# kuetuofa/Transformer

Measured on AMD Instinct MI355X. Metric: tokens/sec (whole node), Transformer-base NMT training, higher is better.
Workload: dtype bf16; 1 GPU; model=transformer-base, num_layers=6, d_model=512, num_heads=8, dff=2048, global_batch=64, seq_len=256, vocab=32770, parallelism=dp1

## Files before the change

transformer_amd/ops/csrc/gemm256.hip:

```cpp
#include "common.h"

#include <torch/extension.h>
#include <ATen/hip/HIPContext.h>

typedef __bf16 bf16x8g __attribute__((ext_vector_type(8)));

namespace {

#define G_BM 256
#define G_BK 64
#define G_THREADS 512
#define G_TILE_ELEMS (G_BM * G_BK)

DEV_INLINE int sw256(int off) { return off ^ (((off >> 9) & 1) << 5); }

template <int ROWS = 256>
DEV_INLINE void stage256(const short* __restrict__ g, long ldg, int row0,
                         int maxrow, int h, short* lds) {
  const int wid = threadIdx.x >> 6, lane = threadIdx.x & 63;
#pragma unroll
  for (int p = 0; p < ROWS / 128; ++p) {
    const int chunk = h * (ROWS / 16) + p * 8 + wid;
    const int d = chunk * 1024 + lane * 16;
    const int lg = sw256(d);
    int row = row0 + (lg >> 7);
    if (row > maxrow - 1) row = maxrow - 1;
    const int colb = lg & 127;
    __builtin_amdgcn_global_load_lds(
        (const __attribute__((address_space(1))) void*)(g + (long)row * ldg +
                                                        (colb >> 1)),
        (__attribute__((address_space(3))) void*)((char*)lds + d), 16, 0, 0);
  }
}

DEV_INLINE bf16x8g frag256(const short* lds, int row, int kb ) {
  const int off = sw256(row * 128 + kb);
  return (bf16x8g)*(const s16x8*)((const char*)lds + off);
}

#define G_BARRIER() __builtin_amdgcn_s_barrier()
#define G_WAIT_LGKM0() asm volatile("s_waitcnt lgkmcnt(0)" ::: "memory")
#define G_WAIT_VM0() asm volatile("s_waitcnt vmcnt(0)" ::: "memory")

template <int EPILOGUE, int BM_, int BN_, int ORDER = 0, int XCDMAP = 1>
__global__ __launch_bounds__(G_THREADS, 1)
void gemm256_kernel(const short* __restrict__ A, const short* __restrict__ B,
                    const short* __restrict__ bias, short* __restrict__ C,
                    int M, int N, int K, int lda, int ldb, int has_bias,
                    int nbm, int nbn, const short* __restrict__ aux) {
  constexpr int MF = BM_ / 32;
  constexpr int NF = BN_ / 64;
  constexpr int A_ELEMS = BM_ * G_BK;
  constexpr int B_ELEMS = BN_ * G_BK;
  constexpr int SLOT = A_ELEMS + B_ELEMS;
  extern __shared__ short smem[];
  const int lane = threadIdx.x & 63;

  int nwg = nbm * nbn;
  int wg = blockIdx.x;
  if (XCDMAP) {
    int q = nwg / 8, r = nwg % 8, x = wg % 8, o = wg / 8;
    wg = (x < r ? x * (q + 1) : r * (q + 1) + (x - r) * q) + o;
  }
  const int bm0 = (ORDER ? (wg % nbm) : (wg / nbn)) * BM_;
  const int bn0 = (ORDER ? (wg / nbm) : (wg % nbn)) * BN_;

  const int wid = threadIdx.x >> 6;
  const int wm = (wid >> 2) * (BM_ / 2);
  const int wn = (wid & 3) * (BN_ / 4);
  const int fr = lane & 15;
  const int kg = lane >> 4;

  f32x4 acc[MF][NF];
#pragma unroll
  for (int i = 0; i < MF; ++i)
#pragma unroll
    for (int j = 0; j < NF; ++j) acc[i][j] = {0.f, 0.f, 0.f, 0.f};

  const int ntiles = K / G_BK;

  {
    short* a0 = smem;
    short* b0 = smem + A_ELEMS;
#pragma unroll
    for (int h = 0; h < 2; ++h) {
      stage256<BM_>(A, lda, bm0, M, h, a0);
      stage256<BN_>(B, ldb, bn0, N, h, b0);
    }
  }
  G_WAIT_VM0();
  G_BARRIER();

  bf16x8g afr[MF / 2][2], bfr[NF][2];

  for (int t = 0; t < ntiles; ++t) {
    const short* a_lds = smem + (t & 1) * SLOT;
    const short* b_lds = a_lds + A_ELEMS;
    short* pa_lds = smem + ((t + 1) & 1) * SLOT;
    short* pb_lds = pa_lds + A_ELEMS;
    const long pk0 = (long)(t + 1) * G_BK;
    const bool do_pf = t + 1 < ntiles;

#define G_MFMA_QUAD(RH, CH)                                                \
  _Pragma("unroll") for (int ks = 0; ks < 2; ++ks)                         \
    _Pragma("unroll") for (int i = 0; i < MF / 2; ++i)                     \
      _Pragma("unroll") for (int j = 0; j < NF / 2; ++j)                   \
        acc[(RH) * (MF / 2) + i][(CH) * (NF / 2) + j] =                    \
            __builtin_amdgcn_mfma_f32_16x16x32_bf16(                       \
                afr[i][ks], bfr[(CH) * (NF / 2) + j][ks],                  \
                acc[(RH) * (MF / 2) + i][(CH) * (NF / 2) + j], 0, 0, 0);

#pragma unroll
    for (int i = 0; i < MF / 2; ++i)
#pragma unroll
      for (int ks = 0; ks < 2; ++ks)
        afr[i][ks] = frag256(a_lds, wm + i * 16 + fr, ks * 64 + kg * 16);
#pragma unroll
    for (int j = 0; j < NF / 2; ++j)
#pragma unroll
      for (int ks = 0; ks < 2; ++ks)
        bfr[j][ks] = frag256(b_lds, wn + j * 16 + fr, ks * 64 + kg * 16);
    if (do_pf) {
      stage256<BM_>(A + pk0, lda, bm0, M, 0, pa_lds);
      stage256<BM_>(A + pk0, lda, bm0, M, 1, pa_lds);
    }
    G_WAIT_LGKM0();
    G_MFMA_QUAD(0, 0)

#pragma unroll
    for (int j = NF / 2; j < NF; ++j)
#pragma unroll
      for (int ks = 0; ks < 2; ++ks)
        bfr[j][ks] = frag256(b_lds, wn + j * 16 + fr, ks * 64 + kg * 16);
    if (do_pf) {
      stage256<BN_>(B + pk0, ldb, bn0, N, 0, pb_lds);
      stage256<BN_>(B + pk0, ldb, bn0, N, 1, pb_lds);
    }
    G_WAIT_LGKM0();
    G_MFMA_QUAD(0, 1)

#pragma unroll
    for (int i = 0; i < MF / 2; ++i)
#pragma unroll
      for (int ks = 0; ks < 2; ++ks)
        afr[i][ks] = frag256(a_lds, wm + (BM_ / 4) + i * 16 + fr,
                             ks * 64 + kg * 16);
    G_WAIT_LGKM0();
    G_MFMA_QUAD(1, 0)

    G_MFMA_QUAD(1, 1)
    G_WAIT_VM0();
    G_BARRIER();
#undef G_MFMA_QUAD
  }

#pragma unroll
  for (int i = 0; i < MF; ++i) {
    const int grow_base = bm0 + wm + i * 16 + kg * 4;
#pragma unroll
    for (int j = 0; j < NF; ++j) {
      const int gcol = bn0 + wn + j * 16 + fr;
      if (gcol >= N) continue;
      const float bv = (has_bias && bias) ? bfbits2f(bias[gcol]) : 0.0f;
#pragma unroll
      for (int r = 0; r < 4; ++r) {
        const int grow = grow_base + r;
        if (grow >= M) continue;
        float v = acc[i][j][r] + bv;
        if (EPILOGUE == 1) v = fmaxf(v, 0.0f);
        if (EPILOGUE == 3) v += bfbits2f(aux[(long)grow * N + gcol]);
        short o = f2bfbits(v);
        if (EPILOGUE == 2)
          o = bfbits2f(aux[(long)grow * N + gcol]) > 0.f ? o : (short)0;
        C[(long)grow * N + gcol] = o;
      }
    }
  }
}

}

static void gemm256_tile(int M, int N, int& BM, int& BN) {
  const long g22 = (long)cdiv(M, 256) * cdiv(N, 256);
  const long g21 = (long)cdiv(M, 256) * cdiv(N, 128);
  auto util = [](long nwg) {
    return nwg < 1 ? 0.0 : (double)nwg / ((nwg + 255) / 256 * 256);
  };
  if (g22 >= 224) {
    BM = 256;
    BN = (util(g21) > util(g22) + 0.1) ? 128 : 256;
  }
  else if (g21 >= 224) { BM = 256; BN = 128; }
  else { BM = 128; BN = 128; }
}

bool gemm256_viable(int M, int N, int K, int lda, int ldb) {
  if (K % G_BK != 0 || K < 2 * G_BK) return false;
  if (lda % 8 != 0 || ldb % 8 != 0) return false;
  int BM, BN;
  gemm256_tile(M, N, BM, BN);
  long nwg = (long)cdiv(M, BM) * cdiv(N, BN);
  return nwg >= 224 && (K >= 512 || nwg >= 384);
}

torch::Tensor gemm256_nt(torch::Tensor a, torch::Tensor w, torch::Tensor bias,
                         int64_t epilogue, c10::optional<torch::Tensor> out,
                         c10::optional<torch::Tensor> aux) {
  TORCH_CHECK(a.is_cuda() && a.dtype() == torch::kBFloat16 && a.dim() == 2 &&
              a.is_contiguous(), "gemm256_nt: a must be contiguous bf16 2-D");
  TORCH_CHECK(w.is_cuda() && w.dtype() == torch::kBFloat16 && w.dim() == 2 &&
              w.is_contiguous(), "gemm256_nt: w must be contiguous bf16 2-D");
  const int M = a.size(0), K = a.size(1), N = w.size(0);
  TORCH_CHECK(w.size(1) == K, "gemm256_nt: K mismatch");
  TORCH_CHECK(K % G_BK == 0 && K >= 2 * G_BK,
              "gemm256_nt: K must be a multiple of 64 (>=128)");
  TORCH_CHECK(epilogue >= 0 && epilogue <= 3, "gemm256_nt: bad epilogue");
  const bool has_bias = epilogue < 2 && bias.defined() && bias.numel() > 0;
  const short* auxp = nullptr;
  if (epilogue >= 2) {
    TORCH_CHECK(aux.has_value() && aux->is_cuda() &&
                aux->dtype() == torch::kBFloat16 && aux->dim() == 2 &&
                aux->is_contiguous() && aux->size(0) == M &&
                aux->size(1) == N,
                "gemm256_nt: epilogue 2/3 needs a contiguous bf16 (M, N) aux");
    TORCH_CHECK(!(bias.defined() && bias.numel() > 0),
                "gemm256_nt: epilogue 2/3 takes no bias");
    auxp = (const short*)aux->data_ptr();
  }
  torch::Tensor c;
  if (out.has_value()) {
    c = *out;
    TORCH_CHECK(c.is_cuda() && c.dtype() == torch::kBFloat16 &&
                c.is_contiguous() && c.numel() == (long)M * N,
                "out must be contiguous bf16 with M*N elements");
    TORCH_CHECK(!auxp || c.data_ptr() != (void*)auxp,
                "gemm256_nt: out must not alias aux");
  } else {
    c = torch::empty({M, N}, a.options());
  }
  int BMv, BNv;
  gemm256_tile(M, N, BMv, BNv);
  const int nbm = cdiv(M, BMv), nbn = cdiv(N, BNv);
  const size_t smem = 2 * ((size_t)BMv + BNv) * G_BK * sizeof(short);
  auto stream = at::hip::getCurrentHIPStream();
  static bool attr_set[4][3] = {};
  static const int env_order = [] {
    const char* e = getenv("TFMX_G256_ORDER");
    return e ? (e[0] == 'n' ? 1 : 0) : -1;
  }();
  static const int env_xcd = [] {
    const char* e = getenv("TFMX_G256_XCD");
    return e ? atoi(e) : -1;
  }();
  const int order = env_order >= 0 ? env_order : 0;
  const int xcd = env_xcd >= 0 ? env_xcd : 1;
  auto launch = [&](auto epi, auto bmc, auto bnc) {
    constexpr int E = decltype(epi)::value;
    constexpr int BM_ = decltype(bmc)::value;
    constexpr int BN_ = decltype(bnc)::value;
    constexpr int ti = BM_ == 128 ? 2 : (BN_ == 128 ? 1 : 0);
    auto go = [&](auto oc, auto xc) {
      constexpr int OV = decltype(oc)::value;
      constexpr int XV = decltype(xc)::value;
      if (!attr_set[E][ti]) {
        (void)hipFuncSetAttribute(
            (const void*)gemm256_kernel<E, BM_, BN_, OV, XV>,
            hipFuncAttributeMaxDynamicSharedMemorySize, (int)smem);
        attr_set[E][ti] = true;
      }
      gemm256_kernel<E, BM_, BN_, OV, XV>
          <<<nbm * nbn, G_THREADS, smem, stream>>>(
              (const short*)a.data_ptr(), (const short*)w.data_ptr(),
              has_bias ? (const short*)bias.data_ptr() : nullptr,
              (short*)c.data_ptr(), M, N, K, K, K, has_bias, nbm, nbn,
              auxp);
    };
    using I0 = std::integral_constant<int, 0>;
    using I1 = std::integral_constant<int, 1>;
    if (order) { if (xcd) go(I1{}, I1{}); else go(I1{}, I0{}); }
    else       { if (xcd) go(I0{}, I1{}); else go(I0{}, I0{}); }
  };
  using E0 = std::integral_constant<int, 0>;
  using E1 = std::integral_constant<int, 1>;
  using E2 = std::integral_constant<int, 2>;
  using E3 = std::integral_constant<int, 3>;
  using T256 = std::integral_constant<int, 256>;
  using T128 = std::integral_constant<int, 128>;
  auto dis = [&](auto epi) {
    if (BMv == 128) launch(epi, T128{}, T128{});
    else if (BNv == 128) launch(epi, T256{}, T128{});
    else launch(epi, T256{}, T256{});
  };
  if (epilogue == 3) dis(E3{});
  else if (epilogue == 2) dis(E2{});
  else if (epilogue == 1) dis(E1{});
  else dis(E0{});
  return c;
}
```

Baseline: 1.868 million tokens/s.

## Vectorize GEMM epilogue via transposed MFMA and LDS-staged 16-byte stores

Swaps the MFMA operand order so each lane holds four consecutive output columns, then writes the epilogue with packed vector stores. By default (aligned, N%8==0) the fragments are staged through a swizzled per-wave LDS slice and written back as 16-byte row-contiguous stores, with bias and aux loads vectorized too. This targets the scalar 2-byte strided global stores of the old epilogue. The cost is extra LDS traffic, more register pressure and more template instances, with a scalar fallback for unaligned shapes.

```diff
diff --git a/transformer_amd/ops/csrc/gemm256.hip b/transformer_amd/ops/csrc/gemm256.hip
--- a/transformer_amd/ops/csrc/gemm256.hip
+++ b/transformer_amd/ops/csrc/gemm256.hip
@@ -1,4 +1,7 @@
 #include "common.h"
+
+#include <cstdint>
+#include <cstring>
 
 #include <torch/extension.h>
 #include <ATen/hip/HIPContext.h>
@@ -38,16 +41,104 @@
   return (bf16x8g)*(const s16x8*)((const char*)lds + off);
 }
 
+DEV_INLINE unsigned pk_bf16(float lo, float hi) {
+  return (unsigned)(unsigned short)f2bfbits(lo) |
+         ((unsigned)(unsigned short)f2bfbits(hi) << 16);
+}
+
+template <int VEC>
+DEV_INLINE f32x4 epi_bias4(const short* __restrict__ bias, int gcol, int N) {
+  f32x4 bv = {0.f, 0.f, 0.f, 0.f};
+  if (bias && gcol < N) {
+    if (VEC == 8) {
+      const s16x4 b = *(const s16x4*)(bias + gcol);
+#pragma unroll
+      for (int r = 0; r < 4; ++r) bv[r] = bfbits2f(b[r]);
+    } else {
+#pragma unroll
+      for (int r = 0; r < 4; ++r)
+        if (gcol + r < N) bv[r] = bfbits2f(bias[gcol + r]);
+    }
+  }
+  return bv;
+}
+
+template <int EPILOGUE, int VEC>
+DEV_INLINE s16x4 epi_frag_value(f32x4 a, f32x4 bv,
+                                const short* __restrict__ aux, long idx,
+                                int gcol, int N) {
+  s16x4 ax = {0, 0, 0, 0};
+  if (EPILOGUE >= 2) {
+    if (VEC == 8) {
+      ax = *(const s16x4*)(aux + idx);
+    } else if (VEC == 2) {
+      const s16x2 lo = *(const s16x2*)(aux + idx);
+      ax[0] = lo[0]; ax[1] = lo[1];
+      if (gcol + 2 < N) {
+        const s16x2 hi = *(const s16x2*)(aux + idx + 2);
+        ax[2] = hi[0]; ax[3] = hi[1];
+      }
+    } else {
+#pragma unroll
+      for (int r = 0; r < 4; ++r)
+        if (gcol + r < N) ax[r] = aux[idx + r];
+    }
+  }
+  float v[4];
+#pragma unroll
+  for (int r = 0; r < 4; ++r) {
+    v[r] = a[r] + bv[r];
+    if (EPILOGUE == 1) v[r] = fmaxf(v[r], 0.0f);
+    if (EPILOGUE == 3) v[r] += bfbits2f(ax[r]);
+  }
+  union { unsigned u[2]; s16x4 s; } o;
+  o.u[0] = pk_bf16(v[0], v[1]);
+  o.u[1] = pk_bf16(v[2], v[3]);
+  if (EPILOGUE == 2) {
+#pragma unroll
+    for (int r = 0; r < 4; ++r)
+      o.s[r] = bfbits2f(ax[r]) > 0.f ? o.s[r] : (short)0;
+  }
+  return o.s;
+}
+
+template <int VEC>
+DEV_INLINE void epi_frag_store(short* __restrict__ C, long idx, int gcol,
+                               int N, s16x4 o) {
+  if (VEC == 8) {
+    *(s16x4*)(C + idx) = o;
+  } else if (VEC == 2) {
+    *(s16x2*)(C + idx) = s16x2{o[0], o[1]};
+    if (gcol + 2 < N) *(s16x2*)(C + idx + 2) = s16x2{o[2], o[3]};
+  } else {
+#pragma unroll
+    for (int r = 0; r < 4; ++r)
+      if (gcol + r < N) C[idx + r] = o[r];
+  }
+}
+
+template <int CW>
+DEV_INLINE int epi_slot16(int row, int q) {
+  return CW == 64 ? row * 128 + ((q ^ (row & 7)) << 4)
+                  : row * 64 + ((q ^ ((row >> 1) & 3)) << 4);
+}
+template <int CW>
+DEV_INLINE int epi_chunk8(int row, int c) {
+  return epi_slot16<CW>(row, c >> 1) + (((c & 1) ^ ((row >> 3) & 1)) << 3);
+}
+
 #define G_BARRIER() __builtin_amdgcn_s_barrier()
 #define G_WAIT_LGKM0() asm volatile("s_waitcnt lgkmcnt(0)" ::: "memory")
 #define G_WAIT_VM0() asm volatile("s_waitcnt vmcnt(0)" ::: "memory")
 
-template <int EPILOGUE, int BM_, int BN_, int ORDER = 0, int XCDMAP = 1>
+template <int EPILOGUE, int BM_, int BN_, int STORE, int ORDER = 0,
+          int XCDMAP = 1>
 __global__ __launch_bounds__(G_THREADS, 1)
 void gemm256_kernel(const short* __restrict__ A, const short* __restrict__ B,
                     const short* __restrict__ bias, short* __restrict__ C,
                     int M, int N, int K, int lda, int ldb, int has_bias,
-                    int nbm, int nbn, const short* __restrict__ aux) {
+                    int nbm, int nbn, const short* __restrict__ aux,
+                    int vec) {
   constexpr int MF = BM_ / 32;
   constexpr int NF = BN_ / 64;
   constexpr int A_ELEMS = BM_ * G_BK;
@@ -107,7 +198,8 @@
       _Pragma("unroll") for (int j = 0; j < NF / 2; ++j)                   \
         acc[(RH) * (MF / 2) + i][(CH) * (NF / 2) + j] =                    \
             __builtin_amdgcn_mfma_f32_16x16x32_bf16(                       \
-                afr[i][ks], bfr[(CH) * (NF / 2) + j][ks],                  \
+                STORE ? bfr[(CH) * (NF / 2) + j][ks] : afr[i][ks],         \
+                STORE ? afr[i][ks] : bfr[(CH) * (NF / 2) + j][ks],         \
                 acc[(RH) * (MF / 2) + i][(CH) * (NF / 2) + j], 0, 0, 0);
 
 #pragma unroll
@@ -154,25 +246,108 @@
 #undef G_MFMA_QUAD
   }
 
-#pragma unroll
-  for (int i = 0; i < MF; ++i) {
-    const int grow_base = bm0 + wm + i * 16 + kg * 4;
-#pragma unroll
-    for (int j = 0; j < NF; ++j) {
-      const int gcol = bn0 + wn + j * 16 + fr;
-      if (gcol >= N) continue;
-      const float bv = (has_bias && bias) ? bfbits2f(bias[gcol]) : 0.0f;
-#pragma unroll
-      for (int r = 0; r < 4; ++r) {
-        const int grow = grow_base + r;
-        if (grow >= M) continue;
-        float v = acc[i][j][r] + bv;
-        if (EPILOGUE == 1) v = fmaxf(v, 0.0f);
-        if (EPILOGUE == 3) v += bfbits2f(aux[(long)grow * N + gcol]);
-        short o = f2bfbits(v);
-        if (EPILOGUE == 2)
-          o = bfbits2f(aux[(long)grow * N + gcol]) > 0.f ? o : (short)0;
-        C[(long)grow * N + gcol] = o;
+  const short* bp = has_bias ? bias : nullptr;
+  if constexpr (STORE == 0) {
+#pragma unroll
+    for (int i = 0; i < MF; ++i) {
+      const int grow_base = bm0 + wm + i * 16 + kg * 4;
+#pragma unroll
+      for (int j = 0; j < NF; ++j) {
+        const int gcol = bn0 + wn + j * 16 + fr;
+        if (gcol >= N) continue;
+        const float bv = bp ? bfbits2f(bp[gcol]) : 0.0f;
+#pragma unroll
+        for (int r = 0; r < 4; ++r) {
+          const int grow = grow_base + r;
+          if (grow >= M) continue;
+          float v = acc[i][j][r] + bv;
+          if (EPILOGUE == 1) v = fmaxf(v, 0.0f);
+          if (EPILOGUE == 3) v += bfbits2f(aux[(long)grow * N + gcol]);
+          short o = f2bfbits(v);
+          if (EPILOGUE == 2)
+            o = bfbits2f(aux[(long)grow * N + gcol]) > 0.f ? o : (short)0;
+          C[(long)grow * N + gcol] = o;
+        }
+      }
+    }
+  } else {
+    auto direct = [&](auto vc) {
+      constexpr int VEC = decltype(vc)::value;
+      f32x4 bv[NF];
+#pragma unroll
+      for (int j = 0; j < NF; ++j)
+        bv[j] = epi_bias4<VEC>(bp, bn0 + wn + j * 16 + kg * 4, N);
+#pragma unroll
+      for (int i = 0; i < MF; ++i) {
+        const int grow = bm0 + wm + i * 16 + fr;
+#pragma unroll
+        for (int j = 0; j < NF; ++j) {
+          const int gcol = bn0 + wn + j * 16 + kg * 4;
+          if (grow >= M || gcol >= N) continue;
+          const long idx = (long)grow * N + gcol;
+          epi_frag_store<VEC>(
+              C, idx, gcol, N,
+              epi_frag_value<EPILOGUE, VEC>(acc[i][j], bv[j], aux, idx, gcol,
+                                            N));
+        }
+      }
+    };
+    using V8 = std::integral_constant<int, 8>;
+    using V2 = std::integral_constant<int, 2>;
+    using V1 = std::integral_constant<int, 1>;
+    if (vec == 2) {
+      direct(V2{});
+    } else if (vec != 8) {
+      direct(V1{});
+    } else if constexpr (STORE == 1) {
+      direct(V8{});
+    } else {
+      constexpr int RW = BM_ / 2, CW = BN_ / 4;
+      constexpr int RPI = 512 / CW;
+      constexpr int NIT = RW / RPI;
+      char* slice = (char*)smem + wid * (RW * CW * 2);
+      f32x4 bv[NF];
+#pragma unroll
+      for (int j = 0; j < NF; ++j)
+        bv[j] = epi_bias4<8>(bp, bn0 + wn + j * 16 + kg * 4, N);
+#pragma unroll
+      for (int i = 0; i < MF; ++i) {
+        const int grow = bm0 + wm + i * 16 + fr;
+#pragma unroll
+        for (int j = 0; j < NF; ++j) {
+          const int gcol = bn0 + wn + j * 16 + kg * 4;
+          const bool in = grow < M && gcol < N;
+          const long idx = in ? (long)grow * N + gcol : 0;
+          const s16x4 o = epi_frag_value<EPILOGUE == 2 ? 0 : EPILOGUE, 8>(
+              acc[i][j], bv[j], aux, idx, gcol, N);
+          *(s16x4*)(slice + epi_chunk8<CW>(i * 16 + fr, j * 4 + kg)) = o;
+        }
+      }
+      const int q = lane & (CW / 8 - 1);
+      const int gcol = bn0 + wn + q * 8;
+      s16x8 ax[EPILOGUE == 2 ? NIT : 1];
+      if (EPILOGUE == 2) {
+#pragma unroll
+        for (int it = 0; it < NIT; ++it) {
+          const int grow = bm0 + wm + it * RPI + lane / (CW / 8);
+          ax[it] = (grow < M && gcol < N)
+                       ? *(const s16x8*)(aux + (long)grow * N + gcol)
+                       : s16x8{0, 0, 0, 0, 0, 0, 0, 0};
+        }
+      }
+      G_WAIT_LGKM0();
+#pragma unroll
+      for (int it = 0; it < NIT; ++it) {
+        const int rr = it * RPI + lane / (CW / 8);
+        const int grow = bm0 + wm + rr;
+        s16x8 o = *(const s16x8*)(slice + epi_slot16<CW>(rr, q));
+        if (rr & 8) o = __builtin_shufflevector(o, o, 4, 5, 6, 7, 0, 1, 2, 3);
+        if (EPILOGUE == 2) {
+#pragma unroll
+          for (int e = 0; e < 8; ++e)
+            o[e] = bfbits2f(ax[it][e]) > 0.f ? o[e] : (short)0;
+        }
+        if (grow < M && gcol < N) *(s16x8*)(C + (long)grow * N + gcol) = o;
       }
     }
   }
@@ -243,7 +418,23 @@
   const int nbm = cdiv(M, BMv), nbn = cdiv(N, BNv);
   const size_t smem = 2 * ((size_t)BMv + BNv) * G_BK * sizeof(short);
   auto stream = at::hip::getCurrentHIPStream();
-  static bool attr_set[4][3] = {};
+  const char* epi_env = getenv("TFMX_G256_EPI");
+  int store = !epi_env ? -2
+              : !strcmp(epi_env, "scalar") ? 0
+              : !strcmp(epi_env, "vec8") ? 1
+              : !strcmp(epi_env, "lds") ? 2 : -1;
+  TORCH_CHECK(store != -1, "TFMX_G256_EPI must be scalar, vec8 or lds");
+  auto aligned = [](const void* p, size_t a) {
+    return p == nullptr || (uintptr_t)p % a == 0;
+  };
+  const void* biasp = has_bias ? bias.data_ptr() : nullptr;
+  int vec = 1;
+  if (N % 8 == 0 && aligned(c.data_ptr(), 16) && aligned(auxp, 16) &&
+      aligned(biasp, 8))
+    vec = 8;
+  else if (N % 2 == 0 && aligned(c.data_ptr(), 4) && aligned(auxp, 4))
+    vec = 2;
+  if (store == -2) store = vec == 8 ? 2 : 0;
   static const int env_order = [] {
     const char* e = getenv("TFMX_G256_ORDER");
     return e ? (e[0] == 'n' ? 1 : 0) : -1;
@@ -258,27 +449,35 @@
     constexpr int E = decltype(epi)::value;
     constexpr int BM_ = decltype(bmc)::value;
     constexpr int BN_ = decltype(bnc)::value;
-    constexpr int ti = BM_ == 128 ? 2 : (BN_ == 128 ? 1 : 0);
-    auto go = [&](auto oc, auto xc) {
+    auto go = [&](auto sc, auto oc, auto xc) {
+      constexpr int SV = decltype(sc)::value;
       constexpr int OV = decltype(oc)::value;
       constexpr int XV = decltype(xc)::value;
-      if (!attr_set[E][ti]) {
+      static bool attr_set = false;
+      if (!attr_set) {
         (void)hipFuncSetAttribute(
-            (const void*)gemm256_kernel<E, BM_, BN_, OV, XV>,
+            (const void*)gemm256_kernel<E, BM_, BN_, SV, OV, XV>,
             hipFuncAttributeMaxDynamicSharedMemorySize, (int)smem);
-        attr_set[E][ti] = true;
-      }
-      gemm256_kernel<E, BM_, BN_, OV, XV>
+        attr_set = true;
+      }
+      gemm256_kernel<E, BM_, BN_, SV, OV, XV>
           <<<nbm * nbn, G_THREADS, smem, stream>>>(
               (const short*)a.data_ptr(), (const short*)w.data_ptr(),
-              has_bias ? (const short*)bias.data_ptr() : nullptr,
-              (short*)c.data_ptr(), M, N, K, K, K, has_bias, nbm, nbn,
-              auxp);
+              (const short*)biasp, (short*)c.data_ptr(), M, N, K, K, K,
+              has_bias, nbm, nbn, auxp, vec);
     };
     using I0 = std::integral_constant<int, 0>;
     using I1 = std::integral_constant<int, 1>;
-    if (order) { if (xcd) go(I1{}, I1{}); else go(I1{}, I0{}); }
-    else       { if (xcd) go(I0{}, I1{}); else go(I0{}, I0{}); }
+    using I2 = std::integral_constant<int, 2>;
+    if (order || !xcd) {
+      TORCH_CHECK(!epi_env || store == 2,
+                  "TFMX_G256_ORDER/XCD probes run on the lds epilogue");
+      if (order) { if (xcd) go(I2{}, I1{}, I1{}); else go(I2{}, I1{}, I0{}); }
+      else go(I2{}, I0{}, I0{});
+    }
+    else if (store == 0) go(I0{}, I0{}, I1{});
+    else if (store == 1) go(I1{}, I0{}, I1{});
+    else go(I2{}, I0{}, I1{});
   };
   using E0 = std::integral_constant<int, 0>;
   using E1 = std::integral_constant<int, 1>;
```

Measured after the change: 1.912 million tokens/s, median of 6. 1.02x the previous value.
